# osqp/OSQP.jl

Hardware: AMD Instinct MI355X
Metric: ADMM iterations/sec (higher is better)
Workload: dtype f64; 1 GPU; rand-1e6; n=1000000, m=1000000, nnz_A=1000000000, nnz_P_full=1000749500, nnz_P_triu=500874750, backend=pcg, check_termination=25, adaptive_rho_interval=50, instances=1

## Files before the change

### osqp.jl_amd/csrc/direct.hip

```cpp
#include <climits>
#include <cstring>
#include <cmath>

#include "engine.hpp"
#include "symbolic.hpp"
#include "mfront.hpp"
#include "mfront_big.hpp"

namespace oq {

namespace {

constexpr int kChainRows = 512;
constexpr int kChainThreads = 1024;

}
}

#include "direct_factor_kernels.hpp"
#include "direct_dense_kernels.hpp"
#include "direct_level_kernels.hpp"
#include "direct_sn_kernels.hpp"
#include "direct_sndense_kernels.hpp"

namespace oq {
namespace {

struct Step { int kind; int a, b, G; int U = 2, L = 64; };

int level_limit();
int64_t factor_limit(const Engine &e, bool forced);
double factor_flops_limit();
struct LdlFactor {
  Engine &e;
  Symbolic S;
  int N = 0, n = 0, mr = 0, nlev = 0;
  double sigma = 0, cconst = 0;
  DevBuf<int64_t> Lp, Rp, Rmap, PtoL, AtoL, Rsplit, Lsplit;
  DevBuf<int> Li, Lcol, Rj, perm, pinv, level_ptr, status;
  DevBuf<double> Lx, Rx, D, Dinv, bp, W, S0a, S0b, x2, gjT, gjW, gjC;
  int lD = 0, cD = 0, kD = 0;
  bool kD_dense = false;
  DevBuf<int> schur_cols;
  int schur_ncols = 0;
  DevBuf<double> dsP1, dsP2;
  double *Sinv = nullptr;
  bool allow_dense_top = true;
  DevBuf<double> S0chk, probe_v, probe_w, probe_r;
  double dense_residual = 0.0;
  static double dense_probe_tol() { const char *v = getenv("OSQP_AMD_DENSE_PROBE_TOL"); return v ? atof(v) : 1e-6; }
  int ldD = 0;
  std::vector<char> long_rows;
  size_t w_half = 0;
  std::vector<Step> fwd, bwd;
  long long factorizations = 0;
  bool sn = false;
  Supernodes T;
  DevBuf<int> sn_ptr, sn_piv, perm_s, pinv_s, sn_Fj, sn_Gi, sn_up, sn_waits, sn_pending, sn_ready;
  int *sn_fault = nullptr, *sn_fault_host = nullptr;
  ~LdlFactor() { if (sn_fault_host) (void)hipHostFree(sn_fault_host); }
  bool faulted() const {
    if (!sn_fault_host) return false;
    if (inject_fault) { inject_fault = false; *sn_fault_host = 1; }
    return *(volatile int *)sn_fault_host != 0;
  }
  mutable bool inject_fault = getenv("OSQP_AMD_SNODE_FAULT_TEST") && atoi(getenv("OSQP_AMD_SNODE_FAULT_TEST")) == 1;
  bool sn_tree = false;
  int sn_tree_threads = 1024;
  int sn_tree_grid = 0;
  DevBuf<int> sn_ticket;
  int sn_tree_L0 = 1;
  DevBuf<int64_t> sn_woff, sn_wmap, sn_Fp, sn_Fpos, sn_Gp, sn_Gpos, sn_Fsplit;
  DevBuf<double> sn_Wc, sn_Wr, sn_Fx, sn_Gx, sn_Dinv;
  std::vector<int> sn_lanes_f, sn_lanes_b;
  bool mf = false;
  DevBuf<int> mf_snof, mf_slot, mf_bsz, mf_chp, mf_chl, mf_list, mf_err;
  DevBuf<int64_t> mf_uoff, mf_reloff;
  DevBuf<uint16_t> mf_rel, mf_loc;
  DevBuf<double> mf_U;
  struct MfLaunch { int cls, off, count, fcap; int tile_off = 0, tile_count = 0, chunk_off = 0, chunk_count = 0; };
  std::vector<MfLaunch> mf_launches;
  DevBuf<int64_t> mf_poff;
  DevBuf<double> mf_panel;
  DevBuf<int64_t> mf_ct0;
  DevBuf<int> mf_tiles, mf_chunks, mf_wide, mf_nwide;
  std::vector<int> mfh_chunks;
  std::vector<int64_t> mfh_poff;
  std::vector<char> mf_is_big;
  std::vector<int> mfh_tiles;
  int mf_big_count = 0, mf_big_fmax = 0;
  int mf_fmax = 0;
  bool mf_ok = false;
  int snd_L0 = -1, snd_J0 = -1, snd_q0 = 0, snd_K = 0;
  int snd_nb = 0, snd_nv = 0, snd_ntiles = 0;
  bool snd_vec_mode = false;
  double snd_skipped = 0.0;
  DevBuf<int> snd_bch, snd_bslot, snd_crange, snd_vptr, snd_tiles, snd_trow_ptr, snd_trow_list, snd_pend_ptr;
  DevBuf<int64_t> snd_boff, snd_pend_src, snd_Fd, snd_vsrc;
  DevBuf<int> snd_dpos, snd_dinv;
  bool lean_built = false;
  std::vector<int> mfh_bsz, mfh_snof, mfh_chp, mfh_chl, mfh_list;
  std::vector<int64_t> mfh_uoff, mfh_reloff;
  const int *vec_perm() const { return sn ? perm_s.get() : perm.get(); }
  const int *vec_pinv() const { return sn ? pinv_s.get() : pinv.get(); }
  int solve_levels() const { return sn ? T.nlev : lD; }
  double flops_below_dense_block() const {
    if (!kD) return S.flops;
    double f = 0.0;
    for (int c = 0; c < cD; c++) { const double cc = (double)(S.Lp[c + 1] - S.Lp[c]); f += cc * cc; }
    return f;
  }

  LdlFactor(Engine &en, const std::vector<int> &row_map, int mr_, double sigma_, double cconst_, int64_t limit,
            double flops_limit = 0.0, bool dense_top = true)
      : e(en), sigma(sigma_), cconst(cconst_), allow_dense_top(dense_top) {
    e.fetch_host_pattern();
    e.setup_mark("  host pattern");
    int first_ordering = getenv("OSQP_AMD_FIRST_ORDERING") ? atoi(getenv("OSQP_AMD_FIRST_ORDERING")) : -1;
    bool nd_by_depth = false;
    const int nd_depth = getenv("OSQP_AMD_ND_DEPTH") ? atoi(getenv("OSQP_AMD_ND_DEPTH")) : 100;
    if (first_ordering < 0 && e.hP.cols + mr_ >= 200000) nd_by_depth = kkt_graph_depth(e.hP, e.hA, row_map, mr_) >= nd_depth;
    if (first_ordering < 0) first_ordering = nd_by_depth ? 1 : 0;
    const int lean_mode = getenv("OSQP_AMD_LEAN") ? atoi(getenv("OSQP_AMD_LEAN")) : -1;
// ... 166 lines not shown
      int per_cu_f = 0, per_cu_b = 0, cus = 0, dev = 0;
      HIP_CHECK(hipGetDevice(&dev));
      HIP_CHECK(hipDeviceGetAttribute(&cus, hipDeviceAttributeMultiprocessorCount, dev));
      per_cu_f = tree_resident((const void *)k_sn_tree<true, 1024>, 1024);
      per_cu_b = tree_resident((const void *)k_sn_tree<false, 1024>, 1024);
      if (const char *v = getenv("OSQP_AMD_SNODE_TREE_PER_CU")) per_cu_f = per_cu_b = std::max(1, atoi(v));
      const int oversub = (mf_ok && mf_big_count > 0) ? (getenv("OSQP_AMD_SNODE_TREE_OVERSUB") ? std::max(1, atoi(getenv("OSQP_AMD_SNODE_TREE_OVERSUB"))) : 2) : 1;
      const long long cap = (long long)oversub * std::min(per_cu_f, per_cu_b) * cus;
      if (getenv("OSQP_AMD_SETUP_TRACE"))
        fprintf(stderr, "[supernodes] one-launch tree: %d / %d resident workgroups of 1024 threads per compute unit (forward / backward), %d compute units, launch of at most %lld\n", per_cu_f, per_cu_b, cus, cap);
      const int top_end = snd_K ? snd_L0 : T.nlev, j_end = snd_K ? snd_J0 : T.count;
      while (sn_tree_L0 < top_end && (long long)(j_end - T.lvl_ptr[sn_tree_L0]) > cap) sn_tree_L0++;
      sn_tree_threads = 1024;
      const bool long_rows = mf_ok && mf_big_count > 0;
      const bool try512 = getenv("OSQP_AMD_SNODE_TREE_512") ? atoi(getenv("OSQP_AMD_SNODE_TREE_512")) != 0 : !long_rows;
      if (sn_tree_L0 > 1 && try512) {
        int pf = 0, pb = 0;
        pf = tree_resident((const void *)k_sn_tree<true, 512>, 512);
        pb = tree_resident((const void *)k_sn_tree<false, 512>, 512);
        if (const char *v = getenv("OSQP_AMD_SNODE_TREE_PER_CU")) pf = pb = 2 * std::max(1, atoi(v));
        long long cap2 = (long long)std::min(pf, pb) * cus;
        if (getenv("OSQP_AMD_SETUP_TRACE")) fprintf(stderr, "[supernodes] one-launch tree: %d / %d resident workgroups of 512 threads per compute unit\n", pf, pb);
        if (getenv("OSQP_AMD_SNODE_TREE_CAP")) cap2 = std::min<long long>(cap2, atoll(getenv("OSQP_AMD_SNODE_TREE_CAP")));
        int L2 = 1;
        while (L2 < top_end && (long long)(j_end - T.lvl_ptr[L2]) > cap2) L2++;
        if (L2 < sn_tree_L0) { sn_tree_L0 = L2; sn_tree_threads = 512; }
        sn_tree_grid = 0;
        int persist_from = 0;
        if (getenv("OSQP_AMD_SNODE_TREE_PERSIST")) persist_from = atoi(getenv("OSQP_AMD_SNODE_TREE_PERSIST"));
        if (persist_from >= 1 && persist_from < sn_tree_L0) {
          sn_tree_L0 = persist_from; sn_tree_threads = 512;
          sn_tree_grid = (int)std::min<long long>(cap2, (long long)(j_end - T.lvl_ptr[sn_tree_L0]));
          sn_ticket.alloc(2);
        }
      }
      if (top_end - sn_tree_L0 < 2) sn_tree = false;
    }
    if (getenv("OSQP_AMD_SETUP_TRACE"))
      fprintf(stderr, "[supernodes] one-launch tree %s: from level %d of %d, %d threads, %d persistent workgroups (0: one per supernode)\n",
              sn_tree ? "on" : "off", sn_tree_L0, T.nlev, sn_tree_threads, sn_tree_grid);
    const int split_level = (sn_tree && sn_tree_L0 > 1) ? sn_tree_L0 : std::min(1, T.nlev);
    const int q_upper = split_level < T.nlev ? T.ptr[T.lvl_ptr[split_level]] : N;
    if (sn_tree && sn_tree_L0 > 1) {
      const int J0 = T.lvl_ptr[sn_tree_L0];
      std::fill(T.waits.begin(), T.waits.end(), 0);
      for (int J = J0; J < T.count; J++)
        if (T.up[J] >= 0) T.waits[T.up[J]]++;
      if (!lean)
        for (int q = 0; q < N; q++)
          T.Fsplit[q] = T.Fp[q] + (std::lower_bound(T.Fj.begin() + T.Fp[q], T.Fj.begin() + T.Fp[q + 1], q_upper) - (T.Fj.begin() + T.Fp[q]));
    }
    up32(sn_up, T.up); up32(sn_waits, T.waits); up32(sn_pending, T.waits);
    sn_ready.alloc(T.count); sn_ready.zero(s);
    if (sn_tree) {
      HIP_CHECK(hipHostMalloc((void **)&sn_fault_host, sizeof(int), hipHostMallocMapped));
      *sn_fault_host = 0;
      HIP_CHECK(hipHostGetDevicePointer((void **)&sn_fault, sn_fault_host, 0));
    }
    up64(sn_woff, T.woff);
    if (lean) lean_device_lists(q_upper);
    else {
      if (!mf_ok) up64(sn_wmap, T.wmap);
      up64(sn_Fp, T.Fp); up64(sn_Fpos, T.Fpos); up64(sn_Gp, T.Gp); up64(sn_Gpos, T.Gpos); up64(sn_Fsplit, T.Fsplit);
    }
    sn_lanes_f.assign(T.nlev, 1); sn_lanes_b.assign(T.nlev, 1);
    for (int L = 0; L < T.nlev; L++) {
      int64_t ef = 0, eb = 0, rows = 0;
      for (int J = T.lvl_ptr[L]; J < T.lvl_ptr[L + 1]; J++) {
        const int q0 = T.ptr[J], q1 = T.ptr[J + 1];
        ef += T.Fp[q1] - T.Fp[q0]; eb += T.Gp[q1] - T.Gp[q0]; rows += q1 - q0;
      }
      sn_lanes_f[L] = pick((double)ef / (double)std::max<int64_t>(1, rows));
      sn_lanes_b[L] = pick((double)eb / (double)std::max<int64_t>(1, rows));
    }
    std::vector<int> ps(N), pis(N);
    for (int q = 0; q < N; q++) { ps[q] = S.perm[T.piv[q]]; pis[ps[q]] = q; }
    up32(perm_s, ps); up32(pinv_s, pis);
    sn_Wc.alloc(T.woff[T.count]); sn_Wr.alloc(T.woff[T.count]);
    sn_Fx.alloc(std::max<size_t>(1, (size_t)T.Fp[N])); sn_Gx.alloc(std::max<size_t>(1, (size_t)T.Gp[N])); sn_Dinv.alloc(N);
    e.sync();
    std::vector<int64_t>().swap(T.wmap); std::vector<int64_t>().swap(T.Fpos); std::vector<int64_t>().swap(T.Gpos);
    std::vector<int>().swap(T.Fj); std::vector<int>().swap(T.Gi);
  }

  int sn_top_Jt = -1, sn_top_level = -1;
  DevBuf<int64_t> sn_Ftop;
  DevBuf<int> sn_tchp, sn_tchl;
  DevBuf<double> sn_uvec;
  SnTop sn_top_args() const {
    if (sn_top_Jt < 0 || !mf) return SnTop{-1, nullptr, nullptr, nullptr, nullptr, nullptr, nullptr, nullptr, nullptr, nullptr};
    return SnTop{sn_top_Jt, sn_Ftop.get(), sn_tchp.get(), sn_tchl.get(), mf_bsz.get(), mf_reloff.get(), mf_rel.get(), mf_poff.get(), mf_panel.get(), sn_uvec.get()};
  }
  void setup_top() {
    sn_top_Jt = -1; sn_top_level = -1;
    if (!mf || !sn_tree || mf_big_count == 0) return;
    if (getenv("OSQP_AMD_SNODE_TOP") && atoi(getenv("OSQP_AMD_SNODE_TOP")) == 0) return;
    if (snd_K && !(getenv("OSQP_AMD_SNODE_TOP") && atoi(getenv("OSQP_AMD_SNODE_TOP")) == 1)) return;
    int Lt = T.nlev;
    for (int L = T.nlev - 1; L >= std::max(1, sn_tree_L0); L--) {
      bool all = true;
      for (int J = T.lvl_ptr[L]; J < T.lvl_ptr[L + 1] && all; J++) all = mfh_poff[J + 1] > mfh_poff[J] && mfh_bsz[J] <= 4096;
      if (!all) break;
      Lt = L;
    }
    if (T.nlev - Lt < 2) return;
    hipStream_t s = e.stream;
    const int Jt = T.lvl_ptr[Lt], q_top = T.ptr[Jt];
    std::vector<int> tchp(T.count - Jt + 1, 0), tchl;
    for (int J = Jt; J < T.count; J++) if (T.up[J] >= 0) tchp[T.up[J] - Jt + 1]++;
    for (int k = 0; k < T.count - Jt; k++) tchp[k + 1] += tchp[k];
    tchl.resize(tchp[T.count - Jt]);
    {
      std::vector<int> fill(tchp.begin(), tchp.end() - 1);
      for (int J = Jt; J < T.count; J++) if (T.up[J] >= 0) tchl[fill[T.up[J] - Jt]++] = J;
    }
    sn_tchp.alloc(tchp.size()); sn_tchp.upload(tchp.data(), tchp.size(), s);
    sn_tchl.alloc(std::max<size_t>(1, tchl.size())); sn_tchl.upload(tchl.data(), tchl.size(), s);
    sn_Ftop.alloc(N);
    OQ_LAUNCH(k_lean_split, dim3(blocks_for(N)), dim3(kBlock), 0, s, N, (const int64_t *)sn_Fp.get(), (const int *)sn_Fj.get(), q_top, sn_Ftop.get());
    sn_uvec.alloc(std::max<int64_t>(1, mfh_reloff[T.count]));
    sn_uvec.zero(s);
    e.sync();
    sn_top_Jt = Jt; sn_top_level = Lt;
    if (getenv("OSQP_AMD_SETUP_TRACE"))
      fprintf(stderr, "[supernodes] top part by front vectors: levels %d .. %d (%d supernodes from %d on; the one-launch tree starts at level %d)\n", Lt,
              T.nlev - 1, T.count - Jt, Jt, sn_tree_L0);
  }

  void setup_dense_top() {
    if (!snd_K) return;
    if (!mf) throw Error(6, "internal: a dense top over the supernodes without the multifrontal plan");
    hipStream_t s = e.stream;
    const int K = snd_K;
    std::vector<int> bch;
    std::vector<int64_t> boff{0};
    for (int J = 0; J < snd_J0; J++)
      if (T.up[J] >= snd_J0 && mfh_bsz[J] > 0) { bch.push_back(J); boff.push_back(boff.back() + mfh_bsz[J]); }
    snd_nb = (int)bch.size();
    auto up32 = [&](DevBuf<int> &d, const std::vector<int> &h) { d.alloc(std::max<size_t>(1, h.size())); d.upload(h.data(), h.size(), s); };
    auto up64 = [&](DevBuf<int64_t> &d, const std::vector<int64_t> &h) { d.alloc(std::max<size_t>(1, h.size())); d.upload(h.data(), h.size(), s); };
    std::vector<int> dpos((size_t)K), dinv((size_t)K);
    {
      const int nd = T.count - snd_J0;
      std::vector<int> order;
// ... 766 lines not shown
  }
#undef OQ_CHAIN_CASE
  void launch_fwd_chain(const Step &t, hipStream_t s) { launch_chain(t, true, s); }
  void launch_bwd_chain(const Step &t, hipStream_t s) { launch_chain(t, false, s); }

#define OQ_SN_LEVEL_W(LA, FWD, GS, JA, JB)                                                                                            \
  OQ_LAUNCH((k_sn_level_w<LA, FWD, GS>), dim3(((JB) - (JA) + 4 * (64 / GS) - 1) / (4 * (64 / GS))), dim3(kSnThreads), 0, s, JA, JB, sn_ptr.get(), \
            sn_woff.get(), FWD ? sn_Fp.get() : sn_Gp.get(), FWD ? sn_Fj.get() : sn_Gi.get(), FWD ? sn_Fx.get() : sn_Gx.get(),          \
            FWD ? sn_Wc.get() : sn_Wr.get(), sn_Dinv.get(), bp.get())
#define OQ_SN_LEVEL(LA, FWD, L)                                                                                                   \
  do {                                                                                                                            \
    const int cnt_ = T.lvl_ptr[L + 1] - T.lvl_ptr[L];                                                                             \
    if (cnt_ >= sn_wave_min_fixed) {                                                                                                \
      const int mid_ = T.lvl_ptr[L] + T.lvl_small[L];                                                                             \
                             \
      const int ones_ = sn_singles ? T.lvl_single[L] : 0, first_ = T.lvl_ptr[L] + ((FWD && L > 0) ? 0 : ones_);                   \
      if (!FWD && ones_ > 0)                                                                                                      \
        OQ_LAUNCH(k_sn_single_bwd, dim3(blocks_for(ones_)), dim3(kBlock), 0, s, T.ptr[T.lvl_ptr[L]], ones_, sn_Gp.get(),          \
                  sn_Gi.get(), sn_Gx.get(), sn_Dinv.get(), bp.get());                                                             \
               \
      if (mid_ > first_) OQ_SN_LEVEL_W((LA == 64 ? 16 : (LA == 16 ? 4 : LA)), FWD, 16, first_, mid_);                             \
      if (T.lvl_ptr[L + 1] > mid_ && !lvl_fold.empty() && lvl_fold[L])                                                            \
        OQ_LAUNCH((k_sn_level_wf<FWD, true>), dim3((T.lvl_ptr[L + 1] - mid_ + 3) / 4), dim3(kSnThreads), 0, s, mid_,               \
                  T.lvl_ptr[L + 1], sn_ptr.get(), sn_woff.get(), FWD ? sn_Fp.get() : sn_Gp.get(), FWD ? sn_Fj.get() : sn_Gi.get(),  \
                  FWD ? sn_Fx.get() : sn_Gx.get(), FWD ? sn_Wc.get() : sn_Wr.get(), sn_Dinv.get(), bp.get());                      \
      else if (T.lvl_ptr[L + 1] > mid_ && sn_flat && !(FWD && L == 0))                                                            \
        OQ_LAUNCH((k_sn_level_wf<FWD, false>), dim3((T.lvl_ptr[L + 1] - mid_ + 3) / 4), dim3(kSnThreads), 0, s, mid_,              \
                  T.lvl_ptr[L + 1], sn_ptr.get(), sn_woff.get(), FWD ? sn_Fp.get() : sn_Gp.get(), FWD ? sn_Fj.get() : sn_Gi.get(),  \
                  FWD ? sn_Fx.get() : sn_Gx.get(), FWD ? sn_Wc.get() : sn_Wr.get(), sn_Dinv.get(), bp.get());                      \
      else if (T.lvl_ptr[L + 1] > mid_) OQ_SN_LEVEL_W((LA == 64 ? 16 : (LA == 16 ? 4 : LA)), FWD, 64, mid_, T.lvl_ptr[L + 1]);     \
    } else if (sn_flat && !lvl_fold.empty() && lvl_fold[L])                                                                       \
      OQ_LAUNCH((k_sn_level_f<FWD, true>), dim3(cnt_), dim3(kSnThreads), 0, s, T.lvl_ptr[L], sn_ptr.get(), sn_woff.get(),          \
                FWD ? sn_Fp.get() : sn_Gp.get(), FWD ? sn_Fj.get() : sn_Gi.get(), FWD ? sn_Fx.get() : sn_Gx.get(),                  \
                FWD ? sn_Wc.get() : sn_Wr.get(), sn_Dinv.get(), bp.get());                                                        \
    else if (sn_flat)                                                                                                             \
      OQ_LAUNCH((k_sn_level_f<FWD, false>), dim3(cnt_), dim3(kSnThreads), 0, s, T.lvl_ptr[L], sn_ptr.get(), sn_woff.get(),         \
                FWD ? sn_Fp.get() : sn_Gp.get(), FWD ? sn_Fj.get() : sn_Gi.get(), FWD ? sn_Fx.get() : sn_Gx.get(),                  \
                FWD ? sn_Wc.get() : sn_Wr.get(), sn_Dinv.get(), bp.get());                                                        \
    else if (cnt_ >= kSnBusyLevel)           \
      OQ_LAUNCH((k_sn_level<(LA == 64 ? 16 : (LA == 16 ? 4 : LA)), FWD>), dim3(cnt_), dim3(kSnThreads), 0, s, T.lvl_ptr[L], sn_ptr.get(), \
                sn_woff.get(), FWD ? sn_Fp.get() : sn_Gp.get(), FWD ? sn_Fj.get() : sn_Gi.get(), FWD ? sn_Fx.get() : sn_Gx.get(),  \
                FWD ? sn_Wc.get() : sn_Wr.get(), sn_Dinv.get(), bp.get());                                                        \
    else                                                                                                                          \
      OQ_LAUNCH((k_sn_level<LA, FWD>), dim3(cnt_), dim3(kSnThreads), 0, s, T.lvl_ptr[L], sn_ptr.get(),                           \
                sn_woff.get(), FWD ? sn_Fp.get() : sn_Gp.get(), FWD ? sn_Fj.get() : sn_Gi.get(), FWD ? sn_Fx.get() : sn_Gx.get(),  \
                FWD ? sn_Wc.get() : sn_Wr.get(), sn_Dinv.get(), bp.get());                                                        \
  } while (0)
#define OQ_SN_TREE(FWD)                                                                                                           \
  if (sn_tree_threads == 512) OQ_SN_TREE_N(FWD, 512); else OQ_SN_TREE_N(FWD, 1024)
#define OQ_SN_TREE_N(FWD, NT_)                                                                                                    \
  OQ_LAUNCH((k_sn_tree<FWD, NT_>), dim3(sn_tree_grid ? sn_tree_grid : sn_j_end() - T.lvl_ptr[sn_tree_L0]), dim3(NT_), 0, s, sn_top_args(), T.lvl_ptr[sn_tree_L0], sn_j_end(), sn_ptr.get(),    \
            sn_woff.get(), FWD ? sn_Fp.get() : sn_Gp.get(), FWD ? sn_Fsplit.get() : sn_Gp.get(), FWD ? sn_Fj.get() : sn_Gi.get(),      \
            FWD ? sn_Fx.get() : sn_Gx.get(), FWD ? sn_Wc.get() : sn_Wr.get(), sn_Dinv.get(), sn_up.get(), sn_waits.get(),          \
            FWD ? sn_pending.get() : sn_ready.get(), sn_fault, bp.get(), sn_tree_grid ? sn_ticket.get() + (FWD ? 0 : 1) : (int *)nullptr)
  const bool sn_fold = !(getenv("OSQP_AMD_SNODE_FOLD") && atoi(getenv("OSQP_AMD_SNODE_FOLD")) == 0) &&
                       !(getenv("OSQP_AMD_SNODE_FLAT") && atoi(getenv("OSQP_AMD_SNODE_FLAT")) == 0);
  const int sn_wave_min_fixed = sn_wave_min();
  const bool sn_fold_wg = !(getenv("OSQP_AMD_SNODE_FOLD") && atoi(getenv("OSQP_AMD_SNODE_FOLD")) == 2);
  std::vector<char> lvl_fold;
  void fold_blocks(hipStream_t s) {
    if (!sn || !sn_fold) return;
    if (lvl_fold.empty()) {
      lvl_fold.assign(T.nlev, 0);
      for (int L = 0; L < T.nlev; L++) {
        const int cnt = T.lvl_ptr[L + 1] - T.lvl_ptr[L], mid = T.lvl_ptr[L] + T.lvl_small[L];
        lvl_fold[L] = (cnt >= sn_wave_min_fixed ? T.lvl_ptr[L + 1] > mid : sn_fold_wg) && !(sn_tree && L >= sn_tree_L0);
      }
    }
    for (int L = 0; L < sn_l_end(); L++) {
      const int cnt = T.lvl_ptr[L + 1] - T.lvl_ptr[L];
      const int mid = cnt >= sn_wave_min_fixed ? T.lvl_ptr[L] + T.lvl_small[L] : T.lvl_ptr[L];
      if (!lvl_fold[L]) continue;
      OQ_LAUNCH(k_sn_fold<true>, dim3(T.lvl_ptr[L + 1] - mid), dim3(64), 0, s, mid, sn_ptr.get(), sn_woff.get(), sn_Wc.get());
      OQ_LAUNCH(k_sn_fold<false>, dim3(T.lvl_ptr[L + 1] - mid), dim3(64), 0, s, mid, sn_ptr.get(), sn_woff.get(), sn_Wr.get());
    }
  }
  const bool sn_flat = !(getenv("OSQP_AMD_SNODE_FLAT") && atoi(getenv("OSQP_AMD_SNODE_FLAT")) == 0);
  const bool sn_singles = !(getenv("OSQP_AMD_SNODE_SINGLE") && atoi(getenv("OSQP_AMD_SNODE_SINGLE")) == 0);
  static int sn_wave_min() { const char *v = getenv("OSQP_AMD_SNODE_WAVE_MIN"); return v ? atoi(v) : kSnWaveLevel; }
  int sn_l_end() const { return snd_K ? snd_L0 : T.nlev; }
  int sn_j_end() const { return snd_K ? snd_J0 : T.count; }
  void run_supernodes() {
    hipStream_t s = e.stream;
    const bool tree = sn_tree && sn_tree_L0 < sn_l_end();
    const int plain = tree ? sn_tree_L0 : sn_l_end();
    for (int L = 0; L < plain; L++) switch (sn_lanes_f[L]) {
      case 1: OQ_SN_LEVEL(1, true, L); break;
      case 4: OQ_SN_LEVEL(4, true, L); break;
      case 16: OQ_SN_LEVEL(16, true, L); break;
      default: OQ_SN_LEVEL(64, true, L); break;
    }
    if (tree && sn_tree_grid) HIP_CHECK(hipMemsetAsync(sn_ticket.get(), 0, 2 * sizeof(int), s));
    if (tree) { OQ_SN_TREE(true); }
    if (snd_K) solve_dense_top(s, tree);
    if (tree) { OQ_SN_TREE(false); }
    for (int L = plain - 1; L >= 0; L--) switch (sn_lanes_b[L]) {
      case 1: OQ_SN_LEVEL(1, false, L); break;
      case 4: OQ_SN_LEVEL(4, false, L); break;
      case 16: OQ_SN_LEVEL(16, false, L); break;
      default: OQ_SN_LEVEL(64, false, L); break;
    }
  }
#undef OQ_SN_LEVEL
#undef OQ_SN_LEVEL_W
#undef OQ_SN_TREE
#undef OQ_SN_TREE_N

  void run_steps(bool skip_first_fwd = false, bool skip_last_bwd = false) {
    hipStream_t s = e.stream;
    if (sn) { run_supernodes(); return; }
    for (size_t si = 0; si < fwd.size(); si++) {
      const Step &t = fwd[si];
      if (si == 0 && skip_first_fwd) continue;
      if (t.kind == 1) {
        const int c0 = S.level_ptr[t.a], c1 = S.level_ptr[t.b];
        if (t.G == kBlock) OQ_LAUNCH(k_fwd_far<kBlock>, dim3(c1 - c0), dim3(kBlock), 0, s, c0, c1, Rp.get(), Rsplit.get(), Rj.get(), Rx.get(), bp.get(), (double *)nullptr);
        else OQ_LAUNCH(k_fwd_far<64>, dim3(blocks_for((int64_t)(c1 - c0) * 64)), dim3(kBlock), 0, s, c0, c1, Rp.get(), Rsplit.get(), Rj.get(), Rx.get(), bp.get(), (double *)nullptr);
        launch_fwd_chain(t, s);
        continue;
      }
      dim3 grid(blocks_for((int64_t)(t.b - t.a) * t.G)), block(kBlock);
      switch (t.G) {
      case 1: OQ_LAUNCH(k_fwd_level<1>, grid, block, 0, s, t.a, t.b, Rp.get(), Rj.get(), Rx.get(), bp.get()); break;
      case 4: OQ_LAUNCH(k_fwd_level<4>, grid, block, 0, s, t.a, t.b, Rp.get(), Rj.get(), Rx.get(), bp.get()); break;
      case 16: OQ_LAUNCH(k_fwd_level<16>, grid, block, 0, s, t.a, t.b, Rp.get(), Rj.get(), Rx.get(), bp.get()); break;
      default: OQ_LAUNCH(k_fwd_level<64>, grid, block, 0, s, t.a, t.b, Rp.get(), Rj.get(), Rx.get(), bp.get()); break;
      }
    }
    if (kD) {
      OQ_LAUNCH(k_fwd_far<kBlock>, dim3(kD), dim3(kBlock), 0, s, cD, N, Rp.get(), Rsplit.get(), Rj.get(), Rx.get(), bp.get(), x2.get());
      if (dsP1.n) {
        const int nb = ldD / kDsT;
        OQ_LAUNCH(k_dense_apply_sym, dim3(nb * (nb + 1) / 2), dim3(256), 0, s, kD, ldD, nb, (const double *)Sinv, (const double *)x2.get(), dsP1.get(), dsP2.get());
        OQ_LAUNCH(k_dense_sym_reduce, dim3(nb), dim3(256), 0, s, kD, nb, (const double *)dsP1.get(), (const double *)dsP2.get(), bp.get() + cD, (const int *)nullptr);
      } else
        OQ_LAUNCH(k_dense_apply, dim3(blocks_for((int64_t)kD * 64)), dim3(kBlock), 0, s, kD, ldD, Sinv, x2.get(), bp.get() + cD);
    }
    for (size_t si = 0; si < bwd.size(); si++) {
      const Step &t = bwd[si];
      if (si + 1 == bwd.size() && skip_last_bwd) continue;
      if (t.kind == 1) {
        const int c0 = S.level_ptr[t.a], c1 = S.level_ptr[t.b];
        if (t.G == kBlock) OQ_LAUNCH(k_bwd_far<kBlock>, dim3(c1 - c0), dim3(kBlock), 0, s, c0, c1, Lsplit.get(), Lp.get(), Li.get(), Lx.get(), Dinv.get(), bp.get());
        else OQ_LAUNCH(k_bwd_far<64>, dim3(blocks_for((int64_t)(c1 - c0) * 64)), dim3(kBlock), 0, s, c0, c1, Lsplit.get(), Lp.get(), Li.get(), Lx.get(), Dinv.get(), bp.get());
        launch_bwd_chain(t, s);
// ... 334 lines not shown
```

### osqp.jl_amd/csrc/direct_sn_kernels.hpp

```cpp
#pragma once
#include "engine.hpp"

namespace oq {
namespace {

constexpr int kSnMax = 64, kSnThreads = 256;
constexpr int kSnBusyLevel = 2048;
constexpr int kSnWaveLevel = 16384;

__global__ __launch_bounds__(kSnThreads) void k_sn_invert(const int *__restrict__ ptr, const int64_t *__restrict__ woff,
                                                          const int64_t *__restrict__ wmap, const double *__restrict__ Lx,
                                                          double *__restrict__ Wc, double *__restrict__ Wr) {
  __shared__ double Ld[kSnMax * kSnMax], Wd[kSnMax * kSnMax];
  const int J = blockIdx.x, s = ptr[J + 1] - ptr[J];
  const int64_t w0 = woff[J];
  for (int e = threadIdx.x; e < s * s; e += kSnThreads) {
    const int i = e / s, k = e - i * s;
    double v = 0.0;
    if (k < i) { const int64_t t = wmap[w0 + (int64_t)i * (i + 1) / 2 + k]; if (t >= 0) v = Lx[t]; }
    Ld[e] = v;
  }
  __syncthreads();
  if ((int)threadIdx.x < s) {
    const int j = threadIdx.x;
// ... 259 lines not shown
  const int nel = s * (s + 1) / 2, h = (s + 1) >> 1;
  for (int e = gl; e < nel; e += 64) tri[e] = Wj[e];
  __builtin_amdgcn_fence(__ATOMIC_RELEASE, "wavefront");
  __builtin_amdgcn_s_waitcnt(0xc07f);
  __builtin_amdgcn_wave_barrier();
  auto at = [&](int r, int c) { return kForward ? tri[c * s - c * (c - 1) / 2 + (r - c)] : tri[r * (r + 1) / 2 + c]; };
  for (int e = gl; e < (s + 1) * h; e += 64) {
    const int k = e / h, a = e - k * h;
    double v;
    if (kForward) v = k <= a ? at(a, k) : (a != s - 1 - a ? at(s - 1 - a, k - a - 1) : 0.0);
    else v = k <= a ? at(s - 1 - a + k, s - 1 - a) : (a != s - 1 - a ? at(k - 1, a) : 0.0);
    Wj[e] = v;
  }
}

__global__ __launch_bounds__(kBlock) void k_sn_single_bwd(int q0, int count, const int64_t *__restrict__ Gp, const int *__restrict__ Gi,
                                                          const double *__restrict__ Gx, const double *__restrict__ Dinv_s,
                                                          double *__restrict__ b) {
  const int i = blockIdx.x * kBlock + threadIdx.x;
  if (i >= count) return;
  const int q = q0 + i;
  const double acc = gather_dot(Gp[q], Gp[q + 1], 1, Gi, Gx, b);
  b[q] = b[q] * Dinv_s[q] - acc;
}

constexpr long long kSnWaitTicks = 20000000LL;
__device__ __forceinline__ int sn_load(const int *p) { return __hip_atomic_load(p, __ATOMIC_RELAXED, __HIP_MEMORY_SCOPE_AGENT); }
template <bool kCoherent>
__device__ __forceinline__ double sn_gather(int64_t i0, int64_t i1, int lane, int la, const int *__restrict__ Ej,
                                            const double *__restrict__ Ex, const double *b) {
  auto ld = [&](int j) { return kCoherent ? __hip_atomic_load(&b[j], __ATOMIC_RELAXED, __HIP_MEMORY_SCOPE_AGENT) : b[j]; };
  double acc = 0.0;
  int64_t i = i0 + lane;
  for (; i + 3 * (int64_t)la < i1; i += 4 * (int64_t)la) {
    const int j0 = Ej[i], j1 = Ej[i + la], j2 = Ej[i + 2 * la], j3 = Ej[i + 3 * la];
    const double x0 = Ex[i], x1 = Ex[i + la], x2 = Ex[i + 2 * la], x3 = Ex[i + 3 * la];
    const double b0 = ld(j0), b1 = ld(j1), b2 = ld(j2), b3 = ld(j3);
    acc += x0 * b0; acc += x1 * b1; acc += x2 * b2; acc += x3 * b3;
  }
  for (; i < i1; i += la) acc += Ex[i] * ld(Ej[i]);
  return acc;
}
template <int NT> constexpr int kSnCapOf = NT == 1024 ? 24 : 20;
struct SnTop {
  int Jt;
  const int64_t *Et;
  const int *tchp, *tchl;
  const int *bsz;
  const int64_t *reloff;
  const uint16_t *rel;
  const int64_t *poff;
  const double *panel;
  double *uvec;
};

template <bool kForward, int NT>
__global__ __launch_bounds__(NT) void k_sn_tree(SnTop top, int J0, int count, const int *__restrict__ ptr, const int64_t *__restrict__ woff,
                                                            const int64_t *__restrict__ Ep, const int64_t *__restrict__ Es,
                                                            const int *__restrict__ Ej, const double *__restrict__ Ex,
                                                            const double *__restrict__ W, const double *__restrict__ Dinv_s,
                                                            const int *__restrict__ up, const int *__restrict__ waits,
                                                            int *__restrict__ sync, int *__restrict__ fault, double *b, int *ticket) {
  __shared__ double t[kSnMax];
  __shared__ double Wl[kSnMax * kSnMax];
  __shared__ double ysc[kSnMax];
  __shared__ int Js;
  for (int k = ticket ? -1 : (int)blockIdx.x;;) {
  if (ticket) {
    __syncthreads();
    if (threadIdx.x == 0) Js = __hip_atomic_fetch_add(ticket, 1, __ATOMIC_RELAXED, __HIP_MEMORY_SCOPE_AGENT);
    __syncthreads();
    k = Js;
    if (k >= count - J0) break;
  }
  const int J = kForward ? J0 + k : count - 1 - k;
  const int P = up[J];
  const int q0 = ptr[J], s = ptr[J + 1] - q0;
  const int la = s <= NT / 64 ? 64 : (s <= NT / 32 ? 32 : (s <= NT / 16 ? 16 : NT / 64));
  const int lane = threadIdx.x & (la - 1), a = threadIdx.x / la;
  const bool mine = a < s;
  const int q = q0 + (mine ? a : 0);
  double acc0 = (kForward && mine) ? sn_gather<false>(Ep[q], Es[q], lane, la, Ej, Ex, b) : 0.0;
  const bool topmode = kForward && top.Jt >= 0 && J >= top.Jt;
  const int64_t i0 = (kForward ? Es[q] : Ep[q]) + lane, i1 = mine ? (topmode ? top.Et[q] : Ep[q + 1]) : 0;
  constexpr int kSnCap = kSnCapOf<NT>;
  int jj[kSnCap];
  double xx[kSnCap];
#pragma unroll
  for (int u = 0; u < kSnCap; u++) {
    const int64_t i = i0 + (int64_t)u * la;
    const bool in = i < i1;
    jj[u] = in ? Ej[i] : q;
    xx[u] = in ? Ex[i] : 0.0;
  }
  {
    const double *Wj = W + woff[J];
    for (int e = threadIdx.x; e < s * (s + 1) / 2; e += NT) Wl[e] = Wj[e];
  }
  const double own = mine ? (kForward ? b[q] : b[q] * Dinv_s[q]) : 0.0;
  if (threadIdx.x == 0) {
    const long long t0 = wall_clock64();
    if (kForward) {
      for (unsigned spins = 1; sn_load(&sync[J]) != 0; spins++) {
        __builtin_amdgcn_s_sleep(1);
        if ((spins & 255u) == 0 && wall_clock64() - t0 > kSnWaitTicks) { *fault = 1; break; }
      }
      sync[J] = waits[J];
    } else if (P >= 0 && P < count) {
      for (unsigned spins = 1; sn_load(&sync[P]) == 0; spins++) {
        __builtin_amdgcn_s_sleep(1);
        if ((spins & 255u) == 0 && wall_clock64() - t0 > kSnWaitTicks) { *fault = 1; break; }
      }
      __hip_atomic_fetch_sub(&sync[P], 1, __ATOMIC_RELAXED, __HIP_MEMORY_SCOPE_AGENT);
    }
  }
  __syncthreads();
  {
    double bb[kSnCap];
#pragma unroll
    for (int u = 0; u < kSnCap; u++) bb[u] = __hip_atomic_load(&b[jj[u]], __ATOMIC_RELAXED, __HIP_MEMORY_SCOPE_AGENT);
    double acc = 0.0;
#pragma unroll
    for (int u = 0; u < kSnCap; u++) acc += xx[u] * bb[u];
    if (i0 + (int64_t)kSnCap * la < i1) acc += sn_gather<true>(i0 - lane + (int64_t)kSnCap * la, i1, lane, la, Ej, Ex, b);
    acc += acc0;
    for (int o = la >> 1; o > 0; o >>= 1) acc += __shfl_xor(acc, o);
    if (lane == 0 && mine) t[a] = own - acc;
  }
  __syncthreads();
  if (topmode) {
    for (int ci = top.tchp[J - top.Jt]; ci < top.tchp[J - top.Jt + 1]; ci++) {
      const int c = top.tchl[ci], bc = top.bsz[c];
      const uint16_t *rl = top.rel + top.reloff[c];
      const double *uc = top.uvec + top.reloff[c];
      for (int i = threadIdx.x; i < bc; i += NT) {
        const int r = rl[i];
        if (r < s) t[r] -= __hip_atomic_load(&uc[i], __ATOMIC_RELAXED, __HIP_MEMORY_SCOPE_AGENT);
      }
      __syncthreads();
    }
  }
  {
    constexpr int LP = NT / 64;
    const int part = threadIdx.x & (LP - 1), r = threadIdx.x / LP;
    double acc = 0.0;
    if (r < s) {
      if (kForward) { for (int j = part; j <= r; j += LP) acc += Wl[j * s - j * (j - 1) / 2 + (r - j)] * t[j]; }
      else { for (int j = r + part; j < s; j += LP) acc += Wl[j * (j + 1) / 2 + r] * t[j]; }
    }
#pragma unroll
    for (int o = LP / 2; o > 0; o >>= 1) acc += __shfl_xor(acc, o);
    if (part == 0 && r < s) {
      __hip_atomic_store(&b[q0 + r], acc, __ATOMIC_RELAXED, __HIP_MEMORY_SCOPE_AGENT);
      if (topmode) ysc[r] = acc * Dinv_s[q0 + r];
    }
  }
  if (topmode) {
    const int bj = top.bsz[J], f = s + bj;
    if (bj > 0) {
      double *uv = Wl;
      __syncthreads();
      for (int i = threadIdx.x; i < bj; i += NT) uv[i] = 0.0;
      __syncthreads();
      for (int ci = top.tchp[J - top.Jt]; ci < top.tchp[J - top.Jt + 1]; ci++) {
        const int c = top.tchl[ci], bc = top.bsz[c];
        const uint16_t *rl = top.rel + top.reloff[c];
        const double *uc = top.uvec + top.reloff[c];
        for (int i = threadIdx.x; i < bc; i += NT) {
          const int r = rl[i];
          if (r >= s) uv[r - s] += __hip_atomic_load(&uc[i], __ATOMIC_RELAXED, __HIP_MEMORY_SCOPE_AGENT);
        }
        __syncthreads();
      }
      const double *Pn = top.panel + top.poff[J] + s;
      double *uj = top.uvec + top.reloff[J];
      for (int i = threadIdx.x; i < bj; i += NT) {
        double a0 = uv[i], a1 = 0.0, a2 = 0.0, a3 = 0.0;
        int p = 0;
        for (; p + 3 < s; p += 4) {
          a0 += Pn[(int64_t)p * f + i] * ysc[p]; a1 += Pn[(int64_t)(p + 1) * f + i] * ysc[p + 1];
          a2 += Pn[(int64_t)(p + 2) * f + i] * ysc[p + 2]; a3 += Pn[(int64_t)(p + 3) * f + i] * ysc[p + 3];
        }
        for (; p < s; p++) a0 += Pn[(int64_t)p * f + i] * ysc[p];
        __hip_atomic_store(&uj[i], (a0 + a1) + (a2 + a3), __ATOMIC_RELAXED, __HIP_MEMORY_SCOPE_AGENT);
      }
    }
  }
  asm volatile("s_waitcnt vmcnt(0)" ::: "memory");
  __syncthreads();
  if (threadIdx.x == 0) {
    if (kForward) { if (P >= 0 && P < count) __hip_atomic_fetch_sub(&sync[P], 1, __ATOMIC_RELAXED, __HIP_MEMORY_SCOPE_AGENT); }
    else if (waits[J] > 0) __hip_atomic_store(&sync[J], waits[J], __ATOMIC_RELAXED, __HIP_MEMORY_SCOPE_AGENT);
  }
  if (!ticket) break;
  }
}

}
}
```

Baseline: 82.47 iterations/s.

## Gather completed-level contributions early in one-launch supernodal tree solve

Adds per-level completion counters and precomputed per-row level split tables so each supernode in the one-launch triangular solve tree can gather contributions from already finished levels while it still waits for its direct dependency. Only the last level's entries stay on the critical path after the wait. This adds level-wide spin waits, extra setup kernels, larger split tables and a per-solve memset. It also includes an optional compile-time profiling path and a dump facility.

Result: slower. 80.67 iterations/s (-2.2%).

```diff
diff --git a/osqp.jl_amd/csrc/direct.hip b/osqp.jl_amd/csrc/direct.hip
--- a/osqp.jl_amd/csrc/direct.hip
+++ b/osqp.jl_amd/csrc/direct.hip
@@ -58,7 +58,57 @@
   Supernodes T;
   DevBuf<int> sn_ptr, sn_piv, perm_s, pinv_s, sn_Fj, sn_Gi, sn_up, sn_waits, sn_pending, sn_ready;
   int *sn_fault = nullptr, *sn_fault_host = nullptr;
-  ~LdlFactor() { if (sn_fault_host) (void)hipHostFree(sn_fault_host); }
+  ~LdlFactor() {
+#ifdef OQ_SN_TREE_PROFILE
+    sn_prof_report();
+#endif
+    if (sn_fault_host) (void)hipHostFree(sn_fault_host);
+  }
+#ifdef OQ_SN_TREE_PROFILE
+  DevBuf<long long> sn_prof;
+  void sn_prof_report() {
+    const char *path = getenv("OSQP_AMD_SN_PROF_OUT");
+    if (!path || !sn_prof.n || !sn_tree) return;
+    if (hipDeviceSynchronize() != hipSuccess) return;
+    std::vector<long long> h(sn_prof.n);
+    if (hipMemcpy(h.data(), sn_prof.get(), h.size() * sizeof(long long), hipMemcpyDeviceToHost) != hipSuccess) return;
+    FILE *f = fopen(path, "a");
+    if (!f) return;
+    const int l_end = sn_l_end();
+    fprintf(f, "# k_sn_tree phases, last solve: N = %d, levels [%d, %d) of %d in the launch, %d supernodes, %d threads, %s\n", N, sn_tree_L0, l_end,
+            T.nlev, sn_j_end() - T.lvl_ptr[sn_tree_L0], sn_tree_threads, sn_tree_grid ? "persistent" : "one workgroup per supernode");
+    fprintf(f, "# us: level = its share of the critical path; entry->wait, gather, product, signal = means over the level's supernodes; last_* = of the supernode that signals last\n");
+    for (int dir = 0; dir < 2; dir++) {
+      auto st = [&](int J, int k) { return h[((size_t)J * 2 + dir) * kSnStamps + k]; };
+      long long first = LLONG_MAX, prev = 0;
+      for (int J = T.lvl_ptr[sn_tree_L0]; J < sn_j_end(); J++) if (st(J, 0)) first = std::min(first, st(J, 0));
+      if (first == LLONG_MAX) continue;
+      prev = first;
+      double tot = 0, tot_g = 0, tot_p = 0, tot_s = 0;
+      fprintf(f, "%s\n dir level  count   level  | waited  gather product  signal | last_gather last_product last_signal  rows_entries\n", dir == 0 ? "forward" : "backward");
+      for (int li = 0; li < l_end - sn_tree_L0; li++) {
+        const int L = dir == 0 ? sn_tree_L0 + li : l_end - 1 - li;
+        const int a = T.lvl_ptr[L], b = T.lvl_ptr[L + 1];
+        long long last = 0; int Jl = a;
+        double w = 0, g = 0, p = 0, sg = 0; int64_t ent = 0;
+        for (int J = a; J < b; J++) {
+          if (st(J, 4) > last) { last = st(J, 4); Jl = J; }
+          w += (double)(st(J, 1) - st(J, 0)); g += (double)(st(J, 2) - st(J, 1)); p += (double)(st(J, 3) - st(J, 2)); sg += (double)(st(J, 4) - st(J, 3));
+          if (T.Fp.size() > (size_t)N && T.Gp.size() > (size_t)N) ent += dir == 0 ? T.Fp[T.ptr[J + 1]] - T.Fp[T.ptr[J]] : T.Gp[T.ptr[J + 1]] - T.Gp[T.ptr[J]];
+        }
+        const double c = 0.01 / (double)(b - a);
+        const double lg = 0.01 * (double)(st(Jl, 2) - st(Jl, 1)), lp = 0.01 * (double)(st(Jl, 3) - st(Jl, 2)), ls = 0.01 * (double)(st(Jl, 4) - st(Jl, 3));
+        fprintf(f, "%4s %5d %6d %7.2f | %6.2f %7.2f %7.2f %7.2f | %11.2f %12.2f %11.2f  %lld\n", dir == 0 ? "fwd" : "bwd", L, b - a, 0.01 * (double)(last - prev),
+                w * c, g * c, p * c, sg * c, lg, lp, ls, (long long)(ent / std::max(1, T.ptr[b] - T.ptr[a])));
+        tot += 0.01 * (double)(last - prev); tot_g += lg; tot_p += lp; tot_s += ls;
+        prev = last;
+      }
+      fprintf(f, "%s total %.2f us; along the last finishers: gather %.2f (%.0f %%), product %.2f, signal %.2f, rest (hand-over latency, entry) %.2f\n", dir == 0 ? "fwd" : "bwd",
+              tot, tot_g, 100.0 * tot_g / std::max(tot, 1e-9), tot_p, tot_s, tot - tot_g - tot_p - tot_s);
+    }
+    fclose(f);
+  }
+#endif
   bool faulted() const {
     if (!sn_fault_host) return false;
     if (inject_fault) { inject_fault = false; *sn_fault_host = 1; }
@@ -69,6 +119,14 @@
   int sn_tree_threads = 1024;
   int sn_tree_grid = 0;
   DevBuf<int> sn_ticket;
+  bool sn_early = false;
+  int sn_early_nl = 0;
+  DevBuf<int> sn_lvl_done, sn_lvl_of, sn_lvl_cnt, sn_lvl_q, sn_lvl_split_f, sn_lvl_split_b;
+  SnEarly sn_early_args(bool fwd) const {
+    if (!sn_early) return SnEarly{nullptr, nullptr, nullptr, nullptr, 0, 0};
+    return SnEarly{fwd ? sn_lvl_split_f.get() : sn_lvl_split_b.get(), sn_lvl_of.get(), sn_lvl_cnt.get(), sn_lvl_done.get() + (fwd ? 0 : sn_early_nl), sn_early_nl,
+                   T.ptr[T.lvl_ptr[sn_tree_L0]]};
+  }
   int sn_tree_L0 = 1;
   DevBuf<int64_t> sn_woff, sn_wmap, sn_Fp, sn_Fpos, sn_Gp, sn_Gpos, sn_Fsplit;
   DevBuf<double> sn_Wc, sn_Wr, sn_Fx, sn_Gx, sn_Dinv;
@@ -341,6 +399,9 @@
     }
     up32(sn_up, T.up); up32(sn_waits, T.waits); up32(sn_pending, T.waits);
     sn_ready.alloc(T.count); sn_ready.zero(s);
+#ifdef OQ_SN_TREE_PROFILE
+    if (sn_tree) { sn_prof.alloc((size_t)T.count * 2 * kSnStamps); sn_prof.zero(s); }
+#endif
     if (sn_tree) {
       HIP_CHECK(hipHostMalloc((void **)&sn_fault_host, sizeof(int), hipHostMallocMapped));
       *sn_fault_host = 0;
@@ -351,6 +412,48 @@
     else {
       if (!mf_ok) up64(sn_wmap, T.wmap);
       up64(sn_Fp, T.Fp); up64(sn_Fpos, T.Fpos); up64(sn_Gp, T.Gp); up64(sn_Gpos, T.Gpos); up64(sn_Fsplit, T.Fsplit);
+    }
+    sn_early = sn_tree && (getenv("OSQP_AMD_SNODE_TREE_EARLY") ? atoi(getenv("OSQP_AMD_SNODE_TREE_EARLY")) != 0 : (mf_ok && mf_big_count > 0));
+    if (sn_early) {
+      const int l_end = snd_K ? snd_L0 : T.nlev, j_end = snd_K ? snd_J0 : T.count, J0 = T.lvl_ptr[sn_tree_L0];
+      const int nl = sn_early_nl = l_end - sn_tree_L0, q0 = T.ptr[J0], rows = T.ptr[j_end] - q0;
+      std::vector<int> lof((size_t)(j_end - J0)), cnt((size_t)nl), ql((size_t)nl + 1);
+      for (int k = 0; k < nl; k++) {
+        cnt[k] = T.lvl_ptr[sn_tree_L0 + k + 1] - T.lvl_ptr[sn_tree_L0 + k];
+        ql[k] = T.ptr[T.lvl_ptr[sn_tree_L0 + k]];
+        for (int J = T.lvl_ptr[sn_tree_L0 + k]; J < T.lvl_ptr[sn_tree_L0 + k + 1]; J++) lof[J - J0] = k;
+      }
+      ql[nl] = T.ptr[j_end];
+      up32(sn_lvl_of, lof); up32(sn_lvl_cnt, cnt); up32(sn_lvl_q, ql);
+      sn_lvl_done.alloc(2 * (size_t)nl); sn_lvl_done.zero(s);
+      const int64_t cells = (int64_t)rows * (nl + 1);
+      sn_lvl_split_f.alloc((size_t)cells); sn_lvl_split_b.alloc((size_t)cells);
+      OQ_LAUNCH(k_sn_lvl_split, dim3(blocks_for(cells)), dim3(kBlock), 0, s, q0, rows, nl, (const int *)sn_lvl_q.get(), (const int64_t *)sn_Fp.get(), (const int *)sn_Fj.get(), sn_lvl_split_f.get());
+      OQ_LAUNCH(k_sn_lvl_split, dim3(blocks_for(cells)), dim3(kBlock), 0, s, q0, rows, nl, (const int *)sn_lvl_q.get(), (const int64_t *)sn_Gp.get(), (const int *)sn_Gi.get(), sn_lvl_split_b.get());
+      if (const char *path = getenv("OSQP_AMD_SNODE_TREE_DUMP")) {
+        e.sync();
+        if (FILE *f = fopen(path, "wb")) {
+          const int64_t f0 = T.Fp[q0], g0 = T.Gp[q0], nf = T.Fp[q0 + rows] - f0, ng = T.Gp[q0 + rows] - g0;
+          const int64_t head[5] = {q0, rows, nl, nf, ng};
+          fwrite(head, sizeof(int64_t), 5, f);
+          fwrite(ql.data(), sizeof(int), ql.size(), f);
+          for (int dir = 0; dir < 2; dir++) {
+            const std::vector<int64_t> &hp = dir == 0 ? T.Fp : T.Gp;
+            const int64_t o = dir == 0 ? f0 : g0, n = dir == 0 ? nf : ng;
+            std::vector<int64_t> pr((size_t)rows + 1);
+            for (int r = 0; r <= rows; r++) pr[r] = hp[q0 + r] - o;
+            std::vector<int> idx((size_t)std::max<int64_t>(1, n)), sp((size_t)cells);
+            if (n) HIP_CHECK(hipMemcpy(idx.data(), (dir == 0 ? sn_Fj.get() : sn_Gi.get()) + o, (size_t)n * sizeof(int), hipMemcpyDeviceToHost));
+            HIP_CHECK(hipMemcpy(sp.data(), dir == 0 ? sn_lvl_split_f.get() : sn_lvl_split_b.get(), (size_t)cells * sizeof(int), hipMemcpyDeviceToHost));
+            fwrite(pr.data(), sizeof(int64_t), pr.size(), f);
+            fwrite(idx.data(), sizeof(int), (size_t)n, f);
+            fwrite(sp.data(), sizeof(int), sp.size(), f);
+          }
+          fclose(f);
+        }
+      }
+      if (getenv("OSQP_AMD_SETUP_TRACE"))
+        fprintf(stderr, "[supernodes] one-launch tree, early gathers: %d levels in the launch, %d rows, level tables of %lld bytes\n", nl, rows, (long long)(2 * cells * (int64_t)sizeof(int)));
     }
     sn_lanes_f.assign(T.nlev, 1); sn_lanes_b.assign(T.nlev, 1);
     for (int L = 0; L < T.nlev; L++) {
@@ -377,8 +480,12 @@
   DevBuf<int> sn_tchp, sn_tchl;
   DevBuf<double> sn_uvec;
   SnTop sn_top_args() const {
-    if (sn_top_Jt < 0 || !mf) return SnTop{-1, nullptr, nullptr, nullptr, nullptr, nullptr, nullptr, nullptr, nullptr, nullptr};
-    return SnTop{sn_top_Jt, sn_Ftop.get(), sn_tchp.get(), sn_tchl.get(), mf_bsz.get(), mf_reloff.get(), mf_rel.get(), mf_poff.get(), mf_panel.get(), sn_uvec.get()};
+    SnTop a{-1, nullptr, nullptr, nullptr, nullptr, nullptr, nullptr, nullptr, nullptr, nullptr};
+    if (sn_top_Jt >= 0 && mf) a = SnTop{sn_top_Jt, sn_Ftop.get(), sn_tchp.get(), sn_tchl.get(), mf_bsz.get(), mf_reloff.get(), mf_rel.get(), mf_poff.get(), mf_panel.get(), sn_uvec.get()};
+#ifdef OQ_SN_TREE_PROFILE
+    a.prof = sn_prof.get();
+#endif
+    return a;
   }
   void setup_top() {
     sn_top_Jt = -1; sn_top_level = -1;
@@ -1251,7 +1358,7 @@
   OQ_LAUNCH((k_sn_tree<FWD, NT_>), dim3(sn_tree_grid ? sn_tree_grid : sn_j_end() - T.lvl_ptr[sn_tree_L0]), dim3(NT_), 0, s, sn_top_args(), T.lvl_ptr[sn_tree_L0], sn_j_end(), sn_ptr.get(),    \
             sn_woff.get(), FWD ? sn_Fp.get() : sn_Gp.get(), FWD ? sn_Fsplit.get() : sn_Gp.get(), FWD ? sn_Fj.get() : sn_Gi.get(),      \
             FWD ? sn_Fx.get() : sn_Gx.get(), FWD ? sn_Wc.get() : sn_Wr.get(), sn_Dinv.get(), sn_up.get(), sn_waits.get(),          \
-            FWD ? sn_pending.get() : sn_ready.get(), sn_fault, bp.get(), sn_tree_grid ? sn_ticket.get() + (FWD ? 0 : 1) : (int *)nullptr)
+            FWD ? sn_pending.get() : sn_ready.get(), sn_fault, bp.get(), sn_tree_grid ? sn_ticket.get() + (FWD ? 0 : 1) : (int *)nullptr, sn_early_args(FWD))
   const bool sn_fold = !(getenv("OSQP_AMD_SNODE_FOLD") && atoi(getenv("OSQP_AMD_SNODE_FOLD")) == 0) &&
                        !(getenv("OSQP_AMD_SNODE_FLAT") && atoi(getenv("OSQP_AMD_SNODE_FLAT")) == 0);
   const int sn_wave_min_fixed = sn_wave_min();
@@ -1290,6 +1397,7 @@
       default: OQ_SN_LEVEL(64, true, L); break;
     }
     if (tree && sn_tree_grid) HIP_CHECK(hipMemsetAsync(sn_ticket.get(), 0, 2 * sizeof(int), s));
+    if (tree && sn_early) HIP_CHECK(hipMemsetAsync(sn_lvl_done.get(), 0, 2 * (size_t)sn_early_nl * sizeof(int), s));
     if (tree) { OQ_SN_TREE(true); }
     if (snd_K) solve_dense_top(s, tree);
     if (tree) { OQ_SN_TREE(false); }
diff --git a/osqp.jl_amd/csrc/direct_sn_kernels.hpp b/osqp.jl_amd/csrc/direct_sn_kernels.hpp
--- a/osqp.jl_amd/csrc/direct_sn_kernels.hpp
+++ b/osqp.jl_amd/csrc/direct_sn_kernels.hpp
@@ -335,7 +335,45 @@
   const int64_t *poff;
   const double *panel;
   double *uvec;
+#ifdef OQ_SN_TREE_PROFILE
+  long long *prof = nullptr;
+#endif
 };
+#ifdef OQ_SN_TREE_PROFILE
+constexpr int kSnStamps = 5;
+#define OQ_SN_STAMP(k_) do { if (threadIdx.x == 0 && top.prof) top.prof[((int64_t)J * 2 + (kForward ? 0 : 1)) * kSnStamps + (k_)] = wall_clock64(); } while (0)
+#else
+#define OQ_SN_STAMP(k_) do { } while (0)
+#endif
+
+__global__ __launch_bounds__(kBlock) void k_sn_lvl_split(int q0, int rows, int nl, const int *__restrict__ lvl_q, const int64_t *__restrict__ Ep,
+                                                         const int *__restrict__ Ej, int *__restrict__ split) {
+  const int64_t i = (int64_t)blockIdx.x * kBlock + threadIdx.x;
+  if (i >= (int64_t)rows * (nl + 1)) return;
+  const int q = q0 + (int)(i / (nl + 1)), bound = lvl_q[i % (nl + 1)];
+  int64_t l = Ep[q], h = Ep[q + 1];
+  while (l < h) { const int64_t mid = (l + h) >> 1; if (Ej[mid] < bound) l = mid + 1; else h = mid; }
+  split[i] = (int)(l - Ep[q]);
+}
+struct SnEarly {
+  const int *split;
+  const int *lvl;
+  const int *cnt;
+  int *done;
+  int nl, q0;
+};
+template <bool kEq>
+__device__ __forceinline__ bool sn_wait(const int *ctr, int want, int *fault) {
+  const long long t0 = wall_clock64();
+  for (unsigned spins = 1; kEq ? sn_load(ctr) != want : sn_load(ctr) == 0; spins++) {
+    __builtin_amdgcn_s_sleep(1);
+    if ((spins & 255u) == 0) {
+      if (wall_clock64() - t0 > kSnWaitTicks) { *fault = 1; return false; }
+      if (*(volatile int *)fault) return false;
+    }
+  }
+  return true;
+}
 
 template <bool kForward, int NT>
 __global__ __launch_bounds__(NT) void k_sn_tree(SnTop top, int J0, int count, const int *__restrict__ ptr, const int64_t *__restrict__ woff,
@@ -343,7 +381,7 @@
                                                             const int *__restrict__ Ej, const double *__restrict__ Ex,
                                                             const double *__restrict__ W, const double *__restrict__ Dinv_s,
                                                             const int *__restrict__ up, const int *__restrict__ waits,
-                                                            int *__restrict__ sync, int *__restrict__ fault, double *b, int *ticket) {
+                                                            int *__restrict__ sync, int *__restrict__ fault, double *b, int *ticket, SnEarly early) {
   __shared__ double t[kSnMax];
   __shared__ double Wl[kSnMax * kSnMax];
   __shared__ double ysc[kSnMax];
@@ -358,6 +396,7 @@
   }
   const int J = kForward ? J0 + k : count - 1 - k;
   const int P = up[J];
+  OQ_SN_STAMP(0);
   const int q0 = ptr[J], s = ptr[J + 1] - q0;
   const int la = s <= NT / 64 ? 64 : (s <= NT / 32 ? 32 : (s <= NT / 16 ? 16 : NT / 64));
   const int lane = threadIdx.x & (la - 1), a = threadIdx.x / la;
@@ -365,7 +404,23 @@
   const int q = q0 + (mine ? a : 0);
   double acc0 = (kForward && mine) ? sn_gather<false>(Ep[q], Es[q], lane, la, Ej, Ex, b) : 0.0;
   const bool topmode = kForward && top.Jt >= 0 && J >= top.Jt;
-  const int64_t i0 = (kForward ? Es[q] : Ep[q]) + lane, i1 = mine ? (topmode ? top.Et[q] : Ep[q + 1]) : 0;
+  int64_t i0 = (kForward ? Es[q] : Ep[q]) + lane, i1 = mine ? (topmode ? top.Et[q] : Ep[q + 1]) : 0;
+  const int lvl = early.split ? early.lvl[J - J0] : 0;
+  if (early.split) {
+    const int *sp = early.split + (int64_t)(q - early.q0) * (early.nl + 1);
+    const int64_t base = Ep[q];
+    const int plvl = kForward ? 0 : ((P >= 0 && P < count) ? early.lvl[P - J0] : early.nl);
+    if (!kForward && mine) {
+      acc0 = sn_gather<false>(base + sp[early.nl], i1, lane, la, Ej, Ex, b);
+    }
+    for (int k = kForward ? 0 : early.nl - 1; kForward ? k < lvl - 1 : k > plvl; k += kForward ? 1 : -1) {
+      if (threadIdx.x == 0) sn_wait<true>(&early.done[k], early.cnt[k], fault);
+      __syncthreads();
+      if (mine) acc0 += sn_gather<true>(std::min(base + sp[k], i1), std::min(base + sp[k + 1], i1), lane, la, Ej, Ex, b);
+    }
+    if (kForward) { if (lvl >= 1) i0 = std::min(base + sp[lvl - 1], i1) + lane; }
+    else i1 = mine ? base + sp[plvl + 1 > early.nl ? early.nl : plvl + 1] : 0;
+  }
   constexpr int kSnCap = kSnCapOf<NT>;
   int jj[kSnCap];
   double xx[kSnCap];
@@ -382,22 +437,14 @@
   }
   const double own = mine ? (kForward ? b[q] : b[q] * Dinv_s[q]) : 0.0;
   if (threadIdx.x == 0) {
-    const long long t0 = wall_clock64();
     if (kForward) {
-      for (unsigned spins = 1; sn_load(&sync[J]) != 0; spins++) {
-        __builtin_amdgcn_s_sleep(1);
-        if ((spins & 255u) == 0 && wall_clock64() - t0 > kSnWaitTicks) { *fault = 1; break; }
-      }
-      sync[J] = waits[J];
+      if (sn_wait<true>(&sync[J], 0, fault)) sync[J] = waits[J];
     } else if (P >= 0 && P < count) {
-      for (unsigned spins = 1; sn_load(&sync[P]) == 0; spins++) {
-        __builtin_amdgcn_s_sleep(1);
-        if ((spins & 255u) == 0 && wall_clock64() - t0 > kSnWaitTicks) { *fault = 1; break; }
-      }
-      __hip_atomic_fetch_sub(&sync[P], 1, __ATOMIC_RELAXED, __HIP_MEMORY_SCOPE_AGENT);
-    }
-  }
-  __syncthreads();
+      if (sn_wait<false>(&sync[P], 0, fault)) __hip_atomic_fetch_sub(&sync[P], 1, __ATOMIC_RELAXED, __HIP_MEMORY_SCOPE_AGENT);
+    }
+  }
+  __syncthreads();
+  OQ_SN_STAMP(1);
   {
     double bb[kSnCap];
 #pragma unroll
@@ -411,6 +458,7 @@
     if (lane == 0 && mine) t[a] = own - acc;
   }
   __syncthreads();
+  OQ_SN_STAMP(2);
   if (topmode) {
     for (int ci = top.tchp[J - top.Jt]; ci < top.tchp[J - top.Jt + 1]; ci++) {
       const int c = top.tchl[ci], bc = top.bsz[c];
@@ -469,12 +517,15 @@
       }
     }
   }
+  OQ_SN_STAMP(3);
   asm volatile("s_waitcnt vmcnt(0)" ::: "memory");
   __syncthreads();
   if (threadIdx.x == 0) {
     if (kForward) { if (P >= 0 && P < count) __hip_atomic_fetch_sub(&sync[P], 1, __ATOMIC_RELAXED, __HIP_MEMORY_SCOPE_AGENT); }
     else if (waits[J] > 0) __hip_atomic_store(&sync[J], waits[J], __ATOMIC_RELAXED, __HIP_MEMORY_SCOPE_AGENT);
-  }
+    if (early.split) __hip_atomic_fetch_add(&early.done[lvl], 1, __ATOMIC_RELAXED, __HIP_MEMORY_SCOPE_AGENT);
+  }
+  OQ_SN_STAMP(4);
   if (!ticket) break;
   }
 }
```
